# augustgw/early-exit-transformer

Measured on AMD Instinct MI355X. Metric: mel-frames/sec encoder forward (all exits) + summed per-exit CTC loss, d_model=256 12-layer, higher is better.
Workload: dtype fp16x3 (hi/lo-split fp16 MFMA operands, three products per GEMM, fp32 accumulate; v_mfma_f32_16x16x32_f16); 1 GPU; early_conformer ctc 12-layer d_model=256 (6 exits x 2), batch 64/GPU, mel [80 x 1027] -> T'=256, log-normal synthetic mel, random-init weights (BASELINE.json configs[1]); global_batch=64, mel_frames=1027, parallelism=dp1 (utterance-batch shards), precision_mode=f16x3

## Files before the change

early_exit_transformer_amd/csrc/ctc.hip:

```cpp
#include <limits.h>

#include "eec_kernels.h"

namespace eec {

constexpr int kCtcPerLane = 8;
constexpr int kCtcEmpty = -(1 << 20);
constexpr float kCtcTiny = 7.52316385e-37f;
constexpr float kCtcRedo = -1.f;
__host__ __device__ inline int ctc_watch_slack(int Tq) {
  int lg = 0;
  while (((long long)Tq * 2048) >> lg) ++lg;
  return 120 - 26 - lg;
}

#define EEC_DPP_F(old, src, ctrl) \
  __builtin_bit_cast(float, __builtin_amdgcn_update_dpp(__builtin_bit_cast(int, (float)(old)), __builtin_bit_cast(int, (float)(src)), ctrl, 0xf, 0xf, false))
#define EEC_DPP_I(old, src, ctrl) __builtin_amdgcn_update_dpp((int)(old), (int)(src), ctrl, 0xf, 0xf, false)

__device__ __forceinline__ size_t ctc_store_index(int lat, int Tq, int P, int t, int k, int lane) {
  return (((size_t)lat * Tq + t) * (P + 1) + k) * 64 + lane;
}

template <int P, bool STORE>
__global__ __launch_bounds__(64) void ctc_alpha_kernel(const float* __restrict__ logp, const long long* __restrict__ targets,
                                                       const long long* __restrict__ target_len, int B, int Tq, int V,
                                                       int S, int blank, float* __restrict__ nll, float* __restrict__ astore) {
  const int lat = blockIdx.x, b = lat % B, lane = threadIdx.x;
  const float* lp = logp + (size_t)lat * Tq * V;
  const long long len_raw = target_len[b];
  bool bad = len_raw < 0 || len_raw > (long long)S;
  const int len = bad ? 0 : (int)len_raw;
  const int L = 2 * len + 1;
  int label[P];
  bool skip_ok[P], live[P];
#pragma unroll
  for (int i = 0; i < P; ++i) {
    const int s = lane * P + i;
    label[i] = blank;
    skip_ok[i] = false;
    live[i] = s < L;
    if (s < L && (s & 1)) {
      const int k = s >> 1;
      const long long lab = targets[(size_t)b * S + k];
      if (lab < 0 || lab >= (long long)V) bad = true;
      label[i] = (lab < 0 || lab >= (long long)V) ? blank : (int)lab;
      skip_ok[i] = k > 0 && lab != targets[(size_t)b * S + k - 1];
    }
  }
  bad = __any((int)bad) != 0;
  float livef[P];
#pragma unroll
  for (int i = 0; i < P; ++i) {
    livef[i] = live[i] ? 1.f : 0.f;
    asm volatile("" : "+v"(label[i]));
  }
  float alpha[P], lim[P];
  int ex = kCtcEmpty;
  static_assert(P % 2 == 0, "a lane's first state must be a blank");
  int eloss = kCtcEmpty;
#pragma unroll
  for (int i = 0; i < P; ++i) {
    const int s = lane * P + i;
    const float l0 = lp[label[i]];
    alpha[i] = (s < 2 && s < L) ? __expf(l0) : 0.f;
    eloss = ((s < 2 && s < L) & (l0 > -INFINITY) & (alpha[i] < kCtcTiny)) ? 0 : eloss;
    lim[i] = live[i] ? -INFINITY : INFINITY;
  }
  if (lane == 0) ex = 0;
  auto store = [&](int t) {
    if constexpr (STORE) {
#pragma unroll
      for (int i = 0; i < P; ++i) astore[ctc_store_index(lat, Tq, P, t, i, lane)] = alpha[i];
      astore[ctc_store_index(lat, Tq, P, t, P, lane)] = __builtin_bit_cast(float, ex);
    }
  };
  store(0);
  constexpr int kCtcAhead = P <= 4 ? 16 : 8;
  float emit[kCtcAhead][P];
#pragma unroll
  for (int d = 0; d < kCtcAhead; ++d)
#pragma unroll
    for (int i = 0; i < P; ++i) emit[d][i] = lp[(size_t)min(1 + d, Tq - 1) * V + label[i]];
  auto step = [&](const float (&em)[P], bool renorm) {
    float up1 = EEC_DPP_F(0.f, alpha[P - 1], 0x138);
    float up2 = EEC_DPP_F(0.f, alpha[P - 2], 0x138);
    const int ex_up = EEC_DPP_I(ex, ex, 0x138);
    const int ec = max(ex, ex_up);
    const int d_own = max(ex - ec, -200), d_up = max(ex_up - ec, -200);
    const float up1s = ldexpf(up1, d_up), up2s = ldexpf(up2, d_up);
    bool lost = (up1 > 0.f) & (up1s < kCtcTiny);
    up1 = up1s;
    up2 = up2s;
    float cur[P];
#pragma unroll
    for (int i = 0; i < P; ++i) {
      cur[i] = ldexpf(alpha[i], d_own);
      lost |= (alpha[i] > 0.f) & (cur[i] < kCtcTiny);
    }
    ex = ec;
#pragma unroll
    for (int i = 0; i < P; ++i) {
      const float p1 = i >= 1 ? cur[i - 1] : up1;
      const float p2 = i >= 2 ? cur[i - 2] : (i == 1 ? up1 : up2);
      const float sum = cur[i] + p1 + (skip_ok[i] ? p2 : 0.f);
      alpha[i] = sum * (__expf(em[i]) * livef[i]);
      lost |= (sum > 0.f) & (alpha[i] < kCtcTiny) & (em[i] > lim[i]);
    }
    eloss = lost ? max(eloss, ec) : eloss;
    if (renorm) {
      float m = alpha[0];
#pragma unroll
      for (int i = 1; i < P; ++i) m = fmaxf(m, alpha[i]);
      const bool any = m > 0.f;
      const int e = any ? (int)((__builtin_bit_cast(unsigned, m) >> 23) & 0xffu) - 127 : 0;
#pragma unroll
      for (int i = 0; i < P; ++i) alpha[i] = ldexpf(alpha[i], -e);
      ex = any ? ex + e : kCtcEmpty;
    }
  };
  int t0 = 1;
  for (; t0 + kCtcAhead <= Tq; t0 += kCtcAhead) {
#pragma unroll
    for (int d = 0; d < kCtcAhead; ++d) {
      step(emit[d], (d & 1) != 0);
      store(t0 + d);
      const int tn = min(t0 + d + kCtcAhead, Tq - 1);
#pragma unroll
      for (int i = 0; i < P; ++i) emit[d][i] = lp[(size_t)tn * V + label[i]];
    }
  }
#pragma unroll
  for (int d = 0; d < kCtcAhead; ++d)
    if (t0 + d < Tq) {
      step(emit[d], (d & 1) != 0);
      store(t0 + d);
    }
  float tail = 0.f;
#pragma unroll
  for (int i = 0; i < P; ++i) {
    const int s = lane * P + i;
    if (s == L - 1 || s == L - 2) tail += alpha[i];
  }
  bad = bad || __any((int)(tail != tail)) != 0;
  const int e_lane = tail > 0.f ? ex : kCtcEmpty;
  const int e_max = (int)wave_max((float)e_lane);
  const float total = wave_sum(tail > 0.f ? ldexpf(tail, max(e_lane - e_max, -200)) : 0.f);
  const int e_tot = total > 0.f ? e_max + (int)((__builtin_bit_cast(unsigned, total) >> 23) & 0xffu) - 127 : 2 * kCtcEmpty;
  const bool redo = __any((int)(eloss > kCtcEmpty && eloss > e_tot + ctc_watch_slack(Tq))) != 0;
  if (lane == 0)
    nll[lat] = (bad || total != total) ? __builtin_nanf("")
               : redo                  ? -INFINITY
               : (total > 0.f)         ? -(logf(total) + (float)e_max * 0.6931471805599453f)
                                       : INFINITY;
  if constexpr (STORE) {
    if (lane == 0) {
      float* pinfo = astore + ctc_store_index(gridDim.x, Tq, P, 0, 0, 0) + 2 * (size_t)lat;
      pinfo[0] = (bad || total != total) ? __builtin_nanf("") : redo ? kCtcRedo : total;
      pinfo[1] = __builtin_bit_cast(float, e_max);
    }
  }
}

template <int P>
__global__ __launch_bounds__(64) void ctc_beta_kernel(const float* __restrict__ logp, const long long* __restrict__ targets,
                                                      const long long* __restrict__ target_len, int B, int Tq, int V,
                                                      int S, int blank, const float* __restrict__ nll, float* __restrict__ astore) {
  const int lat = blockIdx.x, b = lat % B, lane = threadIdx.x;
  const float* lp = logp + (size_t)lat * Tq * V;
  float* pinfo = astore + ctc_store_index(gridDim.x, Tq, P, 0, 0, 0) + 2 * (size_t)lat;
  if (pinfo[0] < 0.f) return;
  const long long len_raw = target_len[b];
  const int len = (len_raw < 0 || len_raw > (long long)S) ? 0 : (int)len_raw;
  const int L = 2 * len + 1;
  int label[P];
  bool skip_ok[P];
  float livef[P], lim[P];
  bool redo = false;
#pragma unroll
  for (int i = 0; i < P; ++i) {
    const int s = lane * P + i;
    label[i] = blank;
    skip_ok[i] = false;
    livef[i] = s < L ? 1.f : 0.f;
    lim[i] = s < L ? -INFINITY : INFINITY;
    if (s < L && (s & 1)) {
      const int k = s >> 1;
      const long long lab = targets[(size_t)b * S + k];
      label[i] = (lab < 0 || lab >= (long long)V) ? blank : (int)lab;
      skip_ok[i] = k > 0 && lab != targets[(size_t)b * S + k - 1];
    }
    asm volatile("" : "+v"(label[i]));
  }
  bool skip_dn[P];
  {
    const int n0 = EEC_DPP_I(0, (int)skip_ok[0], 0x130), n1 = EEC_DPP_I(0, (int)skip_ok[1], 0x130);
#pragma unroll
    for (int i = 0; i < P; ++i) skip_dn[i] = i + 2 < P ? skip_ok[i + 2] : ((i + 2 - P == 0 ? n0 : n1) != 0);
  }
  const float ptot = pinfo[0];
  const bool usable = ptot > 0.f && ptot < INFINITY;
  const int ishift = usable ? -__builtin_bit_cast(int, pinfo[1]) : 0;
  const float fscale = usable ? 1.0f / ptot : 0.f;
  const int e_ptot = (int)((__builtin_bit_cast(unsigned, ptot) >> 23) & 0xffu) - 127;
  const int e_harm = usable ? -ishift + e_ptot + ctc_watch_slack(Tq) : INT_MAX;
  const int sh_harm = 120 - 26 - 2 + e_ptot;
  float beta[P];
  int eb = kCtcEmpty;
  bool any0 = false;
#pragma unroll
  for (int i = 0; i < P; ++i) {
    const int s = lane * P + i;
    beta[i] = (s < L && (s == L - 1 || s == L - 2)) ? 1.f : 0.f;
    any0 = any0 || beta[i] != 0.f;
  }
  if (any0) eb = 0;
  constexpr int kAhead = P <= 4 ? 8 : 4;
  float emit[kAhead][P], al[kAhead][P + 1];
  auto fetch = [&](int slot, int t) {
    const int tc = max(t, 0);
#pragma unroll
    for (int i = 0; i < P; ++i) emit[slot][i] = lp[(size_t)tc * V + label[i]];
#pragma unroll
    for (int k = 0; k <= P; ++k) al[slot][k] = astore[ctc_store_index(lat, Tq, P, tc, k, lane)];
  };
#pragma unroll
  for (int d = 0; d < kAhead; ++d) fetch(d, Tq - 1 - d);
  auto step = [&](int slot, int t, bool renorm) {
    const int ea = __builtin_bit_cast(int, al[slot][P]);
    const int sh = max(min(ea + eb + ishift, 126), -300);
#pragma unroll
    for (int i = 0; i < P; ++i) {
      const float ab = al[slot][i] * beta[i];
      redo |= (al[slot][i] > 0.f) & (beta[i] > 0.f) & (ab < kCtcTiny) & (sh > sh_harm);
      astore[ctc_store_index(lat, Tq, P, t, i, lane)] = ldexpf(ab * fscale, sh) * livef[i];
    }
    float bw[P];
    bool lost = false;
#pragma unroll
    for (int i = 0; i < P; ++i) {
      bw[i] = beta[i] * (__expf(emit[slot][i]) * livef[i]);
      lost |= (beta[i] > 0.f) & (bw[i] < kCtcTiny) & (emit[slot][i] > lim[i]);
    }
    float dn1 = EEC_DPP_F(0.f, bw[0], 0x130);
    float dn2 = EEC_DPP_F(0.f, bw[1], 0x130);
    const int eb_dn = EEC_DPP_I(kCtcEmpty, eb, 0x130);
    const int ec = max(eb, eb_dn);
    const int d_own = max(eb - ec, -200), d_dn = max(eb_dn - ec, -200);
    const float dn1s = ldexpf(dn1, d_dn), dn2s = ldexpf(dn2, d_dn);
    lost |= ((dn1 > 0.f) & (dn1s < kCtcTiny)) | ((dn2 > 0.f) & (dn2s < kCtcTiny));
    dn1 = dn1s;
    dn2 = dn2s;
#pragma unroll
    for (int i = 0; i < P; ++i) {
      const float sh_own = ldexpf(bw[i], d_own);
      lost |= (bw[i] > 0.f) & (sh_own < kCtcTiny);
      bw[i] = sh_own;
    }
    eb = ec;
    redo |= lost & (ec > e_harm);
#pragma unroll
    for (int i = 0; i < P; ++i) {
      const float n1 = i + 1 < P ? bw[i + 1 < P ? i + 1 : 0] : dn1;
      const float n2 = i + 2 < P ? bw[i + 2 < P ? i + 2 : 0] : (i + 2 - P == 0 ? dn1 : dn2);
      beta[i] = bw[i] + n1 + (skip_dn[i] ? n2 : 0.f);
    }
    if (renorm) {
      float m = beta[0];
#pragma unroll
      for (int i = 1; i < P; ++i) m = fmaxf(m, beta[i]);
      const bool any = m > 0.f;
      const int e = any ? (int)((__builtin_bit_cast(unsigned, m) >> 23) & 0xffu) - 127 : 0;
#pragma unroll
      for (int i = 0; i < P; ++i) beta[i] = ldexpf(beta[i], -e);
      eb = any ? eb + e : kCtcEmpty;
    }
  };
  int t = Tq - 1;
  for (; t - kAhead + 1 >= 0; t -= kAhead) {
#pragma unroll
    for (int d = 0; d < kAhead; ++d) {
      step(d, t - d, (d & 1) != 0);
      fetch(d, t - d - kAhead);
    }
  }
#pragma unroll
  for (int d = 0; d < kAhead; ++d)
    if (t - d >= 0) step(d, t - d, (d & 1) != 0);
  if (usable && __any((int)redo) != 0 && lane == 0) pinfo[0] = kCtcRedo;
}

template <int P>
__global__ __launch_bounds__(256) void ctc_grad_kernel(const float* __restrict__ logp, const long long* __restrict__ targets,
                                                       const long long* __restrict__ target_len, int B, int Tq, int V, int S,
                                                       int blank, const float* __restrict__ nll, const float* __restrict__ astore,
                                                       const float* __restrict__ grad_loss, int n_rows, float* __restrict__ dlogp) {
  __shared__ float bins_all[4][256];
  const int lane = threadIdx.x & 63, w = threadIdx.x >> 6;
  const int row = blockIdx.x * 4 + w;
  float* bins = bins_all[w];
  const bool row_ok = row < n_rows;
  const int lat = row_ok ? row / Tq : 0, t = row_ok ? row - lat * Tq : 0, b = lat % B, e = lat / B;
  *(float4*)(bins + lane * 4) = make_float4(0.f, 0.f, 0.f, 0.f);
  __syncthreads();
  const long long len_raw = target_len[b];
  const int len = (len_raw < 0 || len_raw > (long long)S) ? 0 : (int)len_raw;
  const int L = 2 * len + 1;
  if (row_ok) {
#pragma unroll
    for (int i = 0; i < P; ++i) {
      const int s = lane * P + i;
      if (s < L) {
        int lab = blank;
        if (s & 1) {
          const long long lr = targets[(size_t)b * S + (s >> 1)];
          lab = (lr < 0 || lr >= (long long)V) ? blank : (int)lr;
        }
        atomicAdd(&bins[lab], astore[ctc_store_index(lat, Tq, P, t, i, lane)]);
      }
    }
  }
  __syncthreads();
  if (!row_ok) return;
  const float nl = nll[lat];
  float gs = grad_loss[e] / ((float)B * (float)(len > 0 ? len : 1));
  if (nl != nl) gs = nl;
  else if (!(nl < INFINITY)) gs = 0.f;
  const int c0 = lane * 4;
  if (c0 < V) {
    const size_t off = ((size_t)lat * Tq + t) * V + c0;
    const float4 l = *(const float4*)(logp + off);
    const float4 g = *(const float4*)(bins + c0);
    float4 o;
    o.x = gs * (__expf(l.x) - g.x), o.y = gs * (__expf(l.y) - g.y), o.z = gs * (__expf(l.z) - g.z), o.w = gs * (__expf(l.w) - g.w);
    if (gs == 0.f) o = make_float4(0.f, 0.f, 0.f, 0.f);
    *(float4*)(dlogp + off) = o;
  }
}

constexpr int kCtcWideEmpty = -(1 << 30);

__device__ __forceinline__ void ctc_wide_exp(float l, float& pm, int& k) {
  const float hi = l * 1.44269502f;
  const float lo = fmaf(l, 1.44269502f, -hi) + l * 1.92596299e-8f;
  const float kf = floorf(hi);
  const bool zero = !(l > -3.0e4f);
  pm = zero ? 0.f : exp2f((hi - kf) + lo);
  k = zero ? 0 : (int)kf;
}
__device__ __forceinline__ void ctc_wide_norm(float v, int base, float& m, int& e) {
  const int ex = (int)((__builtin_bit_cast(unsigned, v) >> 23) & 0xffu) - 127;
  const bool any = v > 0.f;
  m = any ? ldexpf(v, -ex) : 0.f;
  e = any ? base + ex : kCtcWideEmpty;
}
__device__ __forceinline__ float ctc_wide_add3(float m0, int e0, float m1, int e1, float m2, int e2, int& ec) {
  ec = max(e0, max(e1, e2));
  return ldexpf(m0, max(e0 - ec, -64)) + ldexpf(m1, max(e1 - ec, -64)) + ldexpf(m2, max(e2 - ec, -64));
}

template <int P, bool GRAD>
__global__ __launch_bounds__(64) void ctc_wide_kernel(const float* __restrict__ logp, const long long* __restrict__ targets,
                                                      const long long* __restrict__ target_len, int B, int Tq, int V, int S,
                                                      int blank, float* __restrict__ nll, float* __restrict__ astore) {
  const int lat = blockIdx.x, b = lat % B, lane = threadIdx.x;
  if constexpr (GRAD) {
    if (!(astore[ctc_store_index(gridDim.x, Tq, P, 0, 0, 0) + 2 * (size_t)lat] < 0.f)) return;
  } else {
    if (!(nll[lat] == -INFINITY)) return;
  }
  const float* lp = logp + (size_t)lat * Tq * V;
  int* estore = GRAD ? (int*)(astore + ctc_store_index(gridDim.x, Tq, P, 0, 0, 0) + 2 * (size_t)gridDim.x) : nullptr;
  const long long len_raw = target_len[b];
  const int len = (len_raw < 0 || len_raw > (long long)S) ? 0 : (int)len_raw;
  const int L = 2 * len + 1;
  int label[P];
  bool skip_ok[P], live[P];
#pragma unroll
  for (int i = 0; i < P; ++i) {
    const int s = lane * P + i;
    label[i] = blank;
    skip_ok[i] = false;
    live[i] = s < L;
    if (s < L && (s & 1)) {
      const int k = s >> 1;
      const long long lab = targets[(size_t)b * S + k];
      label[i] = (lab < 0 || lab >= (long long)V) ? blank : (int)lab;
      skip_ok[i] = k > 0 && lab != targets[(size_t)b * S + k - 1];
    }
  }
  float am[P];
  int ae[P];
#pragma unroll
  for (int i = 0; i < P; ++i) {
    const int s = lane * P + i;
    float pm;
    int k;
    ctc_wide_exp(lp[label[i]], pm, k);
    ctc_wide_norm((s < 2 && s < L) ? pm : 0.f, k, am[i], ae[i]);
  }
  auto store = [&](int t) {
    if constexpr (GRAD) {
#pragma unroll
      for (int i = 0; i < P; ++i) {
        astore[ctc_store_index(lat, Tq, P, t, i, lane)] = am[i];
        estore[(((size_t)lat * Tq + t) * P + i) * 64 + lane] = ae[i];
      }
    }
  };
  store(0);
  constexpr int kAhead = 4;
  float emit[kAhead][P];
#pragma unroll
  for (int d = 0; d < kAhead; ++d)
#pragma unroll
    for (int i = 0; i < P; ++i) emit[d][i] = lp[(size_t)min(1 + d, Tq - 1) * V + label[i]];
  for (int t0 = 1; t0 < Tq; t0 += kAhead)
#pragma unroll
  for (int d = 0; d < kAhead; ++d) {
    const int t = t0 + d;
    if (t >= Tq) break;
    const float u1m = EEC_DPP_F(0.f, am[P - 1], 0x138), u2m = EEC_DPP_F(0.f, am[P - 2], 0x138);
    const int u1e = EEC_DPP_I(kCtcWideEmpty, ae[P - 1], 0x138), u2e = EEC_DPP_I(kCtcWideEmpty, ae[P - 2], 0x138);
    float nm[P];
    int ne[P];
#pragma unroll
    for (int i = 0; i < P; ++i) {
      const float p1m = i >= 1 ? am[i >= 1 ? i - 1 : 0] : u1m;
      const int p1e = i >= 1 ? ae[i >= 1 ? i - 1 : 0] : u1e;
      float p2m = i >= 2 ? am[i >= 2 ? i - 2 : 0] : (i == 1 ? u1m : u2m);
      int p2e = i >= 2 ? ae[i >= 2 ? i - 2 : 0] : (i == 1 ? u1e : u2e);
      if (!skip_ok[i]) p2m = 0.f, p2e = kCtcWideEmpty;
      float pm;
      int k, ec;
      ctc_wide_exp(emit[d][i], pm, k);
      const float sum = ctc_wide_add3(am[i], ae[i], p1m, p1e, p2m, p2e, ec);
      ctc_wide_norm(live[i] ? sum * pm : 0.f, ec + k, nm[i], ne[i]);
    }
#pragma unroll
    for (int i = 0; i < P; ++i) {
      am[i] = nm[i], ae[i] = ne[i];
      emit[d][i] = lp[(size_t)min(t + kAhead, Tq - 1) * V + label[i]];
    }
    store(t);
  }
  float tm = 0.f;
  int te = kCtcWideEmpty;
#pragma unroll
  for (int i = 0; i < P; ++i) {
    const int s = lane * P + i;
    if (s == L - 1 || s == L - 2) {
      int ec;
      tm = ctc_wide_add3(tm, te, am[i], ae[i], 0.f, kCtcWideEmpty, ec);
      te = tm > 0.f ? ec : kCtcWideEmpty;
    }
  }
  int e_max = te;
#pragma unroll
  for (int off = 32; off >= 1; off >>= 1) e_max = max(e_max, __shfl_xor(e_max, off, 64));
  float total = ldexpf(tm, max(te - e_max, -64));
#pragma unroll
  for (int off = 32; off >= 1; off >>= 1) total += __shfl_xor(total, off, 64);
  float mt;
  int et;
  ctc_wide_norm(total, e_max, mt, et);
  if constexpr (!GRAD) {
    if (lane == 0) nll[lat] = total > 0.f ? -(logf(mt) + (float)et * 0.6931471805599453f) : INFINITY;
    return;
  } else {
    if (!(total > 0.f)) return;
    bool skip_dn[P];
    {
      int n0 = __shfl_down((int)skip_ok[0], 1, 64), n1 = __shfl_down((int)skip_ok[1], 1, 64);
      if (lane == 63) n0 = n1 = 0;
#pragma unroll
      for (int i = 0; i < P; ++i) skip_dn[i] = i + 2 < P ? skip_ok[i + 2 < P ? i + 2 : 0] : ((i + 2 - P == 0 ? n0 : n1) != 0);
    }
    const float inv = 1.0f / mt;
    float bm[P];
    int be[P];
#pragma unroll
    for (int i = 0; i < P; ++i) {
      const int s = lane * P + i;
      const bool last = s < L && (s == L - 1 || s == L - 2);
      bm[i] = last ? 1.f : 0.f;
      be[i] = last ? 0 : kCtcWideEmpty;
    }
    for (int t = Tq - 1; t >= 0; --t) {
      float wm[P];
      int we[P];
#pragma unroll
      for (int i = 0; i < P; ++i) {
        const size_t ia = ctc_store_index(lat, Tq, P, t, i, lane);
        const float a_m = astore[ia];
        const int a_e = estore[(((size_t)lat * Tq + t) * P + i) * 64 + lane];
        const bool nz = a_m > 0.f && bm[i] > 0.f;
        const int sh = nz ? min(max(a_e + be[i] - et, -200), 126) : 0;
        astore[ia] = nz ? ldexpf(a_m * bm[i] * inv, sh) : 0.f;
        float pm;
        int k;
        ctc_wide_exp(lp[(size_t)t * V + label[i]], pm, k);
        ctc_wide_norm(live[i] ? bm[i] * pm : 0.f, be[i] + k, wm[i], we[i]);
      }
      float d1m = __shfl_down(wm[0], 1, 64), d2m = __shfl_down(wm[1], 1, 64);
      int d1e = __shfl_down(we[0], 1, 64), d2e = __shfl_down(we[1], 1, 64);
      if (lane == 63) d1m = d2m = 0.f, d1e = d2e = kCtcWideEmpty;
#pragma unroll
      for (int i = 0; i < P; ++i) {
        const float n1m = i + 1 < P ? wm[i + 1 < P ? i + 1 : 0] : d1m;
        const int n1e = i + 1 < P ? we[i + 1 < P ? i + 1 : 0] : d1e;
        float n2m = i + 2 < P ? wm[i + 2 < P ? i + 2 : 0] : (i + 2 - P == 0 ? d1m : d2m);
        int n2e = i + 2 < P ? we[i + 2 < P ? i + 2 : 0] : (i + 2 - P == 0 ? d1e : d2e);
        if (!skip_dn[i]) n2m = 0.f, n2e = kCtcWideEmpty;
        int ec;
        const float sum = ctc_wide_add3(wm[i], we[i], n1m, n1e, n2m, n2e, ec);
        ctc_wide_norm(sum, ec, bm[i], be[i]);
      }
    }
  }
}

int ctc_states_per_lane(int S) {
  if (2 * S + 1 <= 64 * 2) return 2;
  if (2 * S + 1 <= 64 * 4) return 4;
  if (2 * S + 1 <= 64 * kCtcPerLane) return kCtcPerLane;
  return 0;
}

size_t ctc_store_floats(int E, int B, int Tq, int S) {
  const int P = ctc_states_per_lane(S);
  return P ? (size_t)E * B * Tq * (P + 1) * 64 + 2 * (size_t)E * B + (size_t)E * B * Tq * P * 64 : 0;
}

hipError_t launch_ctc_backward(const float* logp, const long long* targets, const long long* target_len, int E, int B, int Tq,
                               int V, int S, int blank, const float* nll, float* astore, const float* grad_loss, float* dlogp,
                               hipStream_t st) {
  const int P = ctc_states_per_lane(S), n_rows = E * B * Tq;
  if (!P || V > 256 || V % 4) return hipErrorInvalidValue;
#define EEC_CTC_BWD(P_)                                                                                                      \
  hipLaunchKernelGGL(ctc_beta_kernel<P_>, dim3(E * B), dim3(64), 0, st, logp, targets, target_len, B, Tq, V, S, blank, nll,  \
                     astore);                                                                                               \
  hipLaunchKernelGGL((ctc_wide_kernel<P_, true>), dim3(E * B), dim3(64), 0, st, logp, targets, target_len, B, Tq, V, S,      \
                     blank, (float*)nullptr, astore);                                                                        \
  hipLaunchKernelGGL(ctc_grad_kernel<P_>, dim3((n_rows + 3) / 4), dim3(256), 0, st, logp, targets, target_len, B, Tq, V, S,  \
                     blank, nll, astore, grad_loss, n_rows, dlogp);
  if (P == 2) {
    EEC_CTC_BWD(2)
  } else if (P == 4) {
    EEC_CTC_BWD(4)
  } else {
    EEC_CTC_BWD(kCtcPerLane)
  }
#undef EEC_CTC_BWD
  return hipGetLastError();
}

__global__ void ctc_reduce_kernel(const float* nll, const long long* target_len, int B, float* out) {
  const int e = blockIdx.x, lane = threadIdx.x;
  float s = 0.f;
  for (int b0 = 0; b0 < B; b0 += 64) {
    const int b = b0 + lane;
    float term = 0.f;
    if (b < B) {
      float v = nll[e * B + b];
      if (isinf(v)) v = 0.f;
      const long long l = target_len[b] > 0 ? target_len[b] : 1;
      term = v / (float)l;
    }
    const int n = min(64, B - b0);
    for (int i = 0; i < n; ++i) s += __shfl(term, i, 64);
  }
  if (lane == 0) out[e] = s / (float)B;
}

hipError_t launch_ctc_loss(const float* logp, const long long* targets, const long long* target_len, int E, int B, int Tq,
                           int V, int S, int blank, float* nll, float* out, float* astore, hipStream_t st) {
  const int P = ctc_states_per_lane(S);
  if (!P) return hipErrorInvalidValue;
#define EEC_CTC_FWD(P_)                                                                                                        \
  if (astore)                                                                                                                  \
    hipLaunchKernelGGL((ctc_alpha_kernel<P_, true>), dim3(E * B), dim3(64), 0, st, logp, targets, target_len, B, Tq, V, S,     \
                       blank, nll, astore);                                                                                    \
  else                                                                                                                         \
    hipLaunchKernelGGL((ctc_alpha_kernel<P_, false>), dim3(E * B), dim3(64), 0, st, logp, targets, target_len, B, Tq, V, S,    \
                       blank, nll, astore);                                                                                    \
  hipLaunchKernelGGL((ctc_wide_kernel<P_, false>), dim3(E * B), dim3(64), 0, st, logp, targets, target_len, B, Tq, V, S,       \
                     blank, nll, astore);
  if (P == 2) {
    EEC_CTC_FWD(2)
  } else if (P == 4) {
    EEC_CTC_FWD(4)
  } else {
    EEC_CTC_FWD(kCtcPerLane)
  }
#undef EEC_CTC_FWD
  hipError_t e = hipGetLastError();
  if (e != hipSuccess) return e;
  hipLaunchKernelGGL(ctc_reduce_kernel, dim3(E), dim3(64), 0, st, nll, target_len, B, out);
  return hipGetLastError();
}

__global__ __launch_bounds__(256) void logsoftmax_bwd_kernel(const float* __restrict__ logp, const float* __restrict__ g, int M, int V,
                                                             float* __restrict__ dlogits) {
  const int lane = threadIdx.x & 63, row = blockIdx.x * 4 + (threadIdx.x >> 6);
  if (row >= M) return;
  const int c0 = lane * 4;
  float4 gv = make_float4(0.f, 0.f, 0.f, 0.f), lv = gv;
  if (c0 < V) {
    gv = *(const float4*)(g + (size_t)row * V + c0);
    lv = *(const float4*)(logp + (size_t)row * V + c0);
  }
  const float sum = wave_sum(gv.x + gv.y + gv.z + gv.w);
  if (c0 < V)
    *(float4*)(dlogits + (size_t)row * V + c0) = make_float4(gv.x - __expf(lv.x) * sum, gv.y - __expf(lv.y) * sum,
                                                             gv.z - __expf(lv.z) * sum, gv.w - __expf(lv.w) * sum);
}

hipError_t launch_logsoftmax_backward(const float* logp, const float* g, int M, int V, float* dlogits, hipStream_t st) {
  if (V > 256 || V % 4) return hipErrorInvalidValue;
  hipLaunchKernelGGL(logsoftmax_bwd_kernel, dim3((M + 3) / 4), dim3(256), 0, st, logp, g, M, V, dlogits);
  return hipGetLastError();
}

}
```

Measured before the change: 19.54 million mel-frames/s.

## Add bidirectional alpha/beta CTC kernel for loss-only forward path

When no alpha store is needed, the forward CTC loss now launches a single 128-thread kernel. One wavefront runs the alpha recursion up to the midpoint while the other runs the beta recursion down from the end, and the two halves are joined through shared memory. This roughly halves the serial time-step chain per utterance and drops the second wide-kernel launch, at the cost of twice the threads per block and a different NaN/invalid handling path. The step logic is also refactored into shared helpers, the beta step now uses DPP instead of shuffles, and a raw exp2 builtin replaces exp2f.

```diff
diff --git a/early_exit_transformer_amd/csrc/ctc.hip b/early_exit_transformer_amd/csrc/ctc.hip
--- a/early_exit_transformer_amd/csrc/ctc.hip
+++ b/early_exit_transformer_amd/csrc/ctc.hip
@@ -339,13 +339,14 @@
 }
 
 constexpr int kCtcWideEmpty = -(1 << 30);
+constexpr int kCtcWideAhead = 4;
 
 __device__ __forceinline__ void ctc_wide_exp(float l, float& pm, int& k) {
   const float hi = l * 1.44269502f;
   const float lo = fmaf(l, 1.44269502f, -hi) + l * 1.92596299e-8f;
   const float kf = floorf(hi);
-  const bool zero = !(l > -3.0e4f);
-  pm = zero ? 0.f : exp2f((hi - kf) + lo);
+  const bool zero = l <= -3.0e4f;
+  pm = zero ? 0.f : __builtin_amdgcn_exp2f((hi - kf) + lo);
   k = zero ? 0 : (int)kf;
 }
 __device__ __forceinline__ void ctc_wide_norm(float v, int base, float& m, int& e) {
@@ -358,6 +359,133 @@
   ec = max(e0, max(e1, e2));
   return ldexpf(m0, max(e0 - ec, -64)) + ldexpf(m1, max(e1 - ec, -64)) + ldexpf(m2, max(e2 - ec, -64));
 }
+
+template <int P>
+__device__ __forceinline__ bool ctc_wide_labels(const long long* __restrict__ targets, const long long* __restrict__ target_len, int b,
+                                                int V, int S, int blank, int lane, int (&label)[P], bool (&skip_ok)[P],
+                                                bool (&live)[P], int& L) {
+  const long long len_raw = target_len[b];
+  bool bad = len_raw < 0 || len_raw > (long long)S;
+  const int len = bad ? 0 : (int)len_raw;
+  L = 2 * len + 1;
+#pragma unroll
+  for (int i = 0; i < P; ++i) {
+    const int s = lane * P + i;
+    label[i] = blank;
+    skip_ok[i] = false;
+    live[i] = s < L;
+    if (s < L && (s & 1)) {
+      const int k = s >> 1;
+      const long long lab = targets[(size_t)b * S + k];
+      bad = bad || lab < 0 || lab >= (long long)V;
+      label[i] = (lab < 0 || lab >= (long long)V) ? blank : (int)lab;
+      skip_ok[i] = k > 0 && lab != targets[(size_t)b * S + k - 1];
+    }
+    asm volatile("" : "+v"(label[i]));
+  }
+  return bad;
+}
+
+template <int P>
+__device__ __forceinline__ void ctc_wide_skip_dn(const bool (&skip_ok)[P], int lane, bool (&skip_dn)[P]) {
+  int n0 = __shfl_down((int)skip_ok[0], 1, 64), n1 = __shfl_down((int)skip_ok[1], 1, 64);
+  if (lane == 63) n0 = n1 = 0;
+#pragma unroll
+  for (int i = 0; i < P; ++i) skip_dn[i] = i + 2 < P ? skip_ok[i + 2 < P ? i + 2 : 0] : ((i + 2 - P == 0 ? n0 : n1) != 0);
+}
+
+template <int P>
+__device__ __forceinline__ void ctc_wide_alpha0(const float* __restrict__ lp, const int (&label)[P], int L, int lane, float (&am)[P],
+                                                int (&ae)[P], bool& nan) {
+#pragma unroll
+  for (int i = 0; i < P; ++i) {
+    const int s = lane * P + i;
+    const float l0 = lp[label[i]];
+    float pm;
+    int k;
+    ctc_wide_exp(l0, pm, k);
+    ctc_wide_norm((s < 2 && s < L) ? pm : 0.f, k, am[i], ae[i]);
+    nan |= s < L && l0 != l0;
+  }
+}
+template <int P>
+__device__ __forceinline__ void ctc_wide_beta_last(int L, int lane, float (&bm)[P], int (&be)[P]) {
+#pragma unroll
+  for (int i = 0; i < P; ++i) {
+    const int s = lane * P + i;
+    const bool last = s < L && (s == L - 1 || s == L - 2);
+    bm[i] = last ? 1.f : 0.f;
+    be[i] = last ? 0 : kCtcWideEmpty;
+  }
+}
+
+template <int P>
+__device__ __forceinline__ void ctc_wide_alpha_step(float (&am)[P], int (&ae)[P], const float (&em)[P], const bool (&skip_ok)[P],
+                                                    const bool (&live)[P], bool& nan) {
+  const float u1m = EEC_DPP_F(0.f, am[P - 1], 0x138), u2m = EEC_DPP_F(0.f, am[P - 2], 0x138);
+  const int u1e = EEC_DPP_I(kCtcWideEmpty, ae[P - 1], 0x138), u2e = EEC_DPP_I(kCtcWideEmpty, ae[P - 2], 0x138);
+  float nm[P];
+  int ne[P];
+#pragma unroll
+  for (int i = 0; i < P; ++i) {
+    const float p1m = i >= 1 ? am[i >= 1 ? i - 1 : 0] : u1m;
+    const int p1e = i >= 1 ? ae[i >= 1 ? i - 1 : 0] : u1e;
+    float p2m = i >= 2 ? am[i >= 2 ? i - 2 : 0] : (i == 1 ? u1m : u2m);
+    int p2e = i >= 2 ? ae[i >= 2 ? i - 2 : 0] : (i == 1 ? u1e : u2e);
+    if (!skip_ok[i]) p2m = 0.f, p2e = kCtcWideEmpty;
+    float pm;
+    int k, ec;
+    ctc_wide_exp(em[i], pm, k);
+    const float sum = ctc_wide_add3(am[i], ae[i], p1m, p1e, p2m, p2e, ec);
+    const float v = live[i] ? sum * pm : 0.f;
+    nan |= v != v;
+    ctc_wide_norm(v, ec + k, nm[i], ne[i]);
+  }
+#pragma unroll
+  for (int i = 0; i < P; ++i) am[i] = nm[i], ae[i] = ne[i];
+}
+
+template <int P>
+__device__ __forceinline__ void ctc_wide_beta_step(float (&bm)[P], int (&be)[P], const float (&em)[P], const bool (&skip_dn)[P],
+                                                   bool& nan) {
+  float wm[P];
+  int we[P];
+#pragma unroll
+  for (int i = 0; i < P; ++i) {
+    float pm;
+    int k;
+    ctc_wide_exp(em[i], pm, k);
+    const float v = bm[i] * pm;
+    nan |= v != v;
+    wm[i] = v > 0.f ? v : 0.f;
+    we[i] = v > 0.f ? be[i] + k : kCtcWideEmpty;
+  }
+  const float d1m = EEC_DPP_F(0.f, wm[0], 0x130), d2m = EEC_DPP_F(0.f, wm[1], 0x130);
+  const int d1e = EEC_DPP_I(kCtcWideEmpty, we[0], 0x130), d2e = EEC_DPP_I(kCtcWideEmpty, we[1], 0x130);
+#pragma unroll
+  for (int i = 0; i < P; ++i) {
+    const float n1m = i + 1 < P ? wm[i + 1 < P ? i + 1 : 0] : d1m;
+    const int n1e = i + 1 < P ? we[i + 1 < P ? i + 1 : 0] : d1e;
+    float n2m = i + 2 < P ? wm[i + 2 < P ? i + 2 : 0] : (i + 2 - P == 0 ? d1m : d2m);
+    int n2e = i + 2 < P ? we[i + 2 < P ? i + 2 : 0] : (i + 2 - P == 0 ? d1e : d2e);
+    if (!skip_dn[i]) n2m = 0.f, n2e = kCtcWideEmpty;
+    int ec;
+    const float sum = ctc_wide_add3(wm[i], we[i], n1m, n1e, n2m, n2e, ec);
+    ctc_wide_norm(sum, ec, bm[i], be[i]);
+  }
+}
+
+__device__ __forceinline__ float ctc_wide_total(float tm, int te, float& mt, int& et) {
+  int e_max = te;
+#pragma unroll
+  for (int off = 32; off >= 1; off >>= 1) e_max = max(e_max, __shfl_xor(e_max, off, 64));
+  float total = ldexpf(tm, max(te - e_max, -64));
+#pragma unroll
+  for (int off = 32; off >= 1; off >>= 1) total += __shfl_xor(total, off, 64);
+  ctc_wide_norm(total, e_max, mt, et);
+  return total;
+}
+
 
 template <int P, bool GRAD>
 __global__ __launch_bounds__(64) void ctc_wide_kernel(const float* __restrict__ logp, const long long* __restrict__ targets,
@@ -371,34 +499,12 @@
   }
   const float* lp = logp + (size_t)lat * Tq * V;
   int* estore = GRAD ? (int*)(astore + ctc_store_index(gridDim.x, Tq, P, 0, 0, 0) + 2 * (size_t)gridDim.x) : nullptr;
-  const long long len_raw = target_len[b];
-  const int len = (len_raw < 0 || len_raw > (long long)S) ? 0 : (int)len_raw;
-  const int L = 2 * len + 1;
-  int label[P];
-  bool skip_ok[P], live[P];
-#pragma unroll
-  for (int i = 0; i < P; ++i) {
-    const int s = lane * P + i;
-    label[i] = blank;
-    skip_ok[i] = false;
-    live[i] = s < L;
-    if (s < L && (s & 1)) {
-      const int k = s >> 1;
-      const long long lab = targets[(size_t)b * S + k];
-      label[i] = (lab < 0 || lab >= (long long)V) ? blank : (int)lab;
-      skip_ok[i] = k > 0 && lab != targets[(size_t)b * S + k - 1];
-    }
-  }
+  int label[P], L;
+  bool skip_ok[P], live[P], nan = false;
+  ctc_wide_labels<P>(targets, target_len, b, V, S, blank, lane, label, skip_ok, live, L);
   float am[P];
   int ae[P];
-#pragma unroll
-  for (int i = 0; i < P; ++i) {
-    const int s = lane * P + i;
-    float pm;
-    int k;
-    ctc_wide_exp(lp[label[i]], pm, k);
-    ctc_wide_norm((s < 2 && s < L) ? pm : 0.f, k, am[i], ae[i]);
-  }
+  ctc_wide_alpha0<P>(lp, label, L, lane, am, ae, nan);
   auto store = [&](int t) {
     if constexpr (GRAD) {
 #pragma unroll
@@ -409,39 +515,19 @@
     }
   };
   store(0);
-  constexpr int kAhead = 4;
-  float emit[kAhead][P];
-#pragma unroll
-  for (int d = 0; d < kAhead; ++d)
+  float emit[kCtcWideAhead][P];
+#pragma unroll
+  for (int d = 0; d < kCtcWideAhead; ++d)
 #pragma unroll
     for (int i = 0; i < P; ++i) emit[d][i] = lp[(size_t)min(1 + d, Tq - 1) * V + label[i]];
-  for (int t0 = 1; t0 < Tq; t0 += kAhead)
-#pragma unroll
-  for (int d = 0; d < kAhead; ++d) {
+  for (int t0 = 1; t0 < Tq; t0 += kCtcWideAhead)
+#pragma unroll
+  for (int d = 0; d < kCtcWideAhead; ++d) {
     const int t = t0 + d;
     if (t >= Tq) break;
-    const float u1m = EEC_DPP_F(0.f, am[P - 1], 0x138), u2m = EEC_DPP_F(0.f, am[P - 2], 0x138);
-    const int u1e = EEC_DPP_I(kCtcWideEmpty, ae[P - 1], 0x138), u2e = EEC_DPP_I(kCtcWideEmpty, ae[P - 2], 0x138);
-    float nm[P];
-    int ne[P];
-#pragma unroll
-    for (int i = 0; i < P; ++i) {
-      const float p1m = i >= 1 ? am[i >= 1 ? i - 1 : 0] : u1m;
-      const int p1e = i >= 1 ? ae[i >= 1 ? i - 1 : 0] : u1e;
-      float p2m = i >= 2 ? am[i >= 2 ? i - 2 : 0] : (i == 1 ? u1m : u2m);
-      int p2e = i >= 2 ? ae[i >= 2 ? i - 2 : 0] : (i == 1 ? u1e : u2e);
-      if (!skip_ok[i]) p2m = 0.f, p2e = kCtcWideEmpty;
-      float pm;
-      int k, ec;
-      ctc_wide_exp(emit[d][i], pm, k);
-      const float sum = ctc_wide_add3(am[i], ae[i], p1m, p1e, p2m, p2e, ec);
-      ctc_wide_norm(live[i] ? sum * pm : 0.f, ec + k, nm[i], ne[i]);
-    }
-#pragma unroll
-    for (int i = 0; i < P; ++i) {
-      am[i] = nm[i], ae[i] = ne[i];
-      emit[d][i] = lp[(size_t)min(t + kAhead, Tq - 1) * V + label[i]];
-    }
+    ctc_wide_alpha_step<P>(am, ae, emit[d], skip_ok, live, nan);
+#pragma unroll
+    for (int i = 0; i < P; ++i) emit[d][i] = lp[(size_t)min(t + kCtcWideAhead, Tq - 1) * V + label[i]];
     store(t);
   }
   float tm = 0.f;
@@ -455,40 +541,22 @@
       te = tm > 0.f ? ec : kCtcWideEmpty;
     }
   }
-  int e_max = te;
-#pragma unroll
-  for (int off = 32; off >= 1; off >>= 1) e_max = max(e_max, __shfl_xor(e_max, off, 64));
-  float total = ldexpf(tm, max(te - e_max, -64));
-#pragma unroll
-  for (int off = 32; off >= 1; off >>= 1) total += __shfl_xor(total, off, 64);
   float mt;
   int et;
-  ctc_wide_norm(total, e_max, mt, et);
+  const float total = ctc_wide_total(tm, te, mt, et);
   if constexpr (!GRAD) {
     if (lane == 0) nll[lat] = total > 0.f ? -(logf(mt) + (float)et * 0.6931471805599453f) : INFINITY;
     return;
   } else {
     if (!(total > 0.f)) return;
     bool skip_dn[P];
-    {
-      int n0 = __shfl_down((int)skip_ok[0], 1, 64), n1 = __shfl_down((int)skip_ok[1], 1, 64);
-      if (lane == 63) n0 = n1 = 0;
-#pragma unroll
-      for (int i = 0; i < P; ++i) skip_dn[i] = i + 2 < P ? skip_ok[i + 2 < P ? i + 2 : 0] : ((i + 2 - P == 0 ? n0 : n1) != 0);
-    }
+    ctc_wide_skip_dn<P>(skip_ok, lane, skip_dn);
     const float inv = 1.0f / mt;
     float bm[P];
     int be[P];
-#pragma unroll
-    for (int i = 0; i < P; ++i) {
-      const int s = lane * P + i;
-      const bool last = s < L && (s == L - 1 || s == L - 2);
-      bm[i] = last ? 1.f : 0.f;
-      be[i] = last ? 0 : kCtcWideEmpty;
-    }
+    ctc_wide_beta_last<P>(L, lane, bm, be);
     for (int t = Tq - 1; t >= 0; --t) {
-      float wm[P];
-      int we[P];
+      float em[P];
 #pragma unroll
       for (int i = 0; i < P; ++i) {
         const size_t ia = ctc_store_index(lat, Tq, P, t, i, lane);
@@ -497,27 +565,96 @@
         const bool nz = a_m > 0.f && bm[i] > 0.f;
         const int sh = nz ? min(max(a_e + be[i] - et, -200), 126) : 0;
         astore[ia] = nz ? ldexpf(a_m * bm[i] * inv, sh) : 0.f;
-        float pm;
-        int k;
-        ctc_wide_exp(lp[(size_t)t * V + label[i]], pm, k);
-        ctc_wide_norm(live[i] ? bm[i] * pm : 0.f, be[i] + k, wm[i], we[i]);
+        em[i] = lp[(size_t)t * V + label[i]];
       }
-      float d1m = __shfl_down(wm[0], 1, 64), d2m = __shfl_down(wm[1], 1, 64);
-      int d1e = __shfl_down(we[0], 1, 64), d2e = __shfl_down(we[1], 1, 64);
-      if (lane == 63) d1m = d2m = 0.f, d1e = d2e = kCtcWideEmpty;
-#pragma unroll
-      for (int i = 0; i < P; ++i) {
-        const float n1m = i + 1 < P ? wm[i + 1 < P ? i + 1 : 0] : d1m;
-        const int n1e = i + 1 < P ? we[i + 1 < P ? i + 1 : 0] : d1e;
-        float n2m = i + 2 < P ? wm[i + 2 < P ? i + 2 : 0] : (i + 2 - P == 0 ? d1m : d2m);
-        int n2e = i + 2 < P ? we[i + 2 < P ? i + 2 : 0] : (i + 2 - P == 0 ? d1e : d2e);
-        if (!skip_dn[i]) n2m = 0.f, n2e = kCtcWideEmpty;
-        int ec;
-        const float sum = ctc_wide_add3(wm[i], we[i], n1m, n1e, n2m, n2e, ec);
-        ctc_wide_norm(sum, ec, bm[i], be[i]);
+      ctc_wide_beta_step<P>(bm, be, em, skip_dn, nan);
+    }
+  }
+}
+
+template <int P>
+__global__ __launch_bounds__(128) void ctc_bidir_kernel(const float* __restrict__ logp, const long long* __restrict__ targets,
+                                                        const long long* __restrict__ target_len, int B, int Tq, int V, int S,
+                                                        int blank, float* __restrict__ nll) {
+  __shared__ float join_m[P][64];
+  __shared__ int join_e[P][64];
+  __shared__ int join_nan;
+  const int lat = blockIdx.x, b = lat % B, lane = threadIdx.x & 63;
+  const bool down = __builtin_amdgcn_readfirstlane((int)threadIdx.x >> 6) != 0;
+  const float* lp = logp + (size_t)lat * Tq * V;
+  int label[P], L;
+  bool skip_ok[P], live[P], nan = false;
+  const bool bad = ctc_wide_labels<P>(targets, target_len, b, V, S, blank, lane, label, skip_ok, live, L);
+  const int mid = (Tq - 1) / 2;
+  constexpr int kAhead = P <= 4 ? 8 : 4;
+  float xm[P], emit[kAhead][P];
+  int xe[P];
+  if (!down) {
+    ctc_wide_alpha0<P>(lp, label, L, lane, xm, xe, nan);
+#pragma unroll
+    for (int d = 0; d < kAhead; ++d)
+#pragma unroll
+      for (int i = 0; i < P; ++i) emit[d][i] = lp[(size_t)min(1 + d, Tq - 1) * V + label[i]];
+    int t0 = 1;
+    for (; t0 + kAhead - 1 <= mid; t0 += kAhead) {
+#pragma unroll
+      for (int d = 0; d < kAhead; ++d) {
+#pragma unroll
+        for (int i = 0; i < P; ++i) asm volatile("" : "+v"(emit[d][i]) : "v"(xm[0]));
+        ctc_wide_alpha_step<P>(xm, xe, emit[d], skip_ok, live, nan);
+        const int tn = min(t0 + d + kAhead, Tq - 1);
+#pragma unroll
+        for (int i = 0; i < P; ++i) emit[d][i] = lp[(size_t)tn * V + label[i]];
       }
     }
-  }
+#pragma unroll
+    for (int d = 0; d < kAhead; ++d)
+      if (t0 + d <= mid) ctc_wide_alpha_step<P>(xm, xe, emit[d], skip_ok, live, nan);
+  } else {
+    bool skip_dn[P];
+    ctc_wide_skip_dn<P>(skip_ok, lane, skip_dn);
+    ctc_wide_beta_last<P>(L, lane, xm, xe);
+#pragma unroll
+    for (int d = 0; d < kAhead; ++d)
+#pragma unroll
+      for (int i = 0; i < P; ++i) emit[d][i] = lp[(size_t)max(Tq - 1 - d, 0) * V + label[i]];
+    int t0 = Tq - 1;
+    for (; t0 - kAhead + 1 > mid; t0 -= kAhead) {
+#pragma unroll
+      for (int d = 0; d < kAhead; ++d) {
+        ctc_wide_beta_step<P>(xm, xe, emit[d], skip_dn, nan);
+        const int tn = max(t0 - d - kAhead, 0);
+#pragma unroll
+        for (int i = 0; i < P; ++i) emit[d][i] = lp[(size_t)tn * V + label[i]];
+      }
+    }
+#pragma unroll
+    for (int d = 0; d < kAhead; ++d)
+      if (t0 - d > mid) ctc_wide_beta_step<P>(xm, xe, emit[d], skip_dn, nan);
+#pragma unroll
+    for (int i = 0; i < P; ++i) join_m[i][lane] = xm[i], join_e[i][lane] = xe[i];
+    const bool any_nan = __any((int)nan) != 0;
+    if (lane == 0) join_nan = (int)any_nan;
+  }
+  __syncthreads();
+  if (down) return;
+  float tm = 0.f;
+  int te = kCtcWideEmpty;
+#pragma unroll
+  for (int i = 0; i < P; ++i) {
+    float pm;
+    int pe, ec;
+    ctc_wide_norm(xm[i] * join_m[i][lane], 0, pm, pe);
+    pe = pm > 0.f ? pe + xe[i] + join_e[i][lane] : kCtcWideEmpty;
+    tm = ctc_wide_add3(tm, te, pm, pe, 0.f, kCtcWideEmpty, ec);
+    te = tm > 0.f ? ec : kCtcWideEmpty;
+  }
+  float mt;
+  int et;
+  const float total = ctc_wide_total(tm, te, mt, et);
+  const bool invalid = join_nan != 0 || __any((int)(bad || nan)) != 0;
+  if (lane == 0)
+    nll[lat] = invalid ? __builtin_nanf("") : total > 0.f ? -(logf(mt) + (float)et * 0.6931471805599453f) : INFINITY;
 }
 
 int ctc_states_per_lane(int S) {
@@ -578,14 +715,15 @@
   const int P = ctc_states_per_lane(S);
   if (!P) return hipErrorInvalidValue;
 #define EEC_CTC_FWD(P_)                                                                                                        \
-  if (astore)                                                                                                                  \
+  if (astore) {                                                                                                                \
     hipLaunchKernelGGL((ctc_alpha_kernel<P_, true>), dim3(E * B), dim3(64), 0, st, logp, targets, target_len, B, Tq, V, S,     \
                        blank, nll, astore);                                                                                    \
-  else                                                                                                                         \
-    hipLaunchKernelGGL((ctc_alpha_kernel<P_, false>), dim3(E * B), dim3(64), 0, st, logp, targets, target_len, B, Tq, V, S,    \
+    hipLaunchKernelGGL((ctc_wide_kernel<P_, false>), dim3(E * B), dim3(64), 0, st, logp, targets, target_len, B, Tq, V, S,     \
                        blank, nll, astore);                                                                                    \
-  hipLaunchKernelGGL((ctc_wide_kernel<P_, false>), dim3(E * B), dim3(64), 0, st, logp, targets, target_len, B, Tq, V, S,       \
-                     blank, nll, astore);
+  } else {                                                                                                                     \
+    hipLaunchKernelGGL(ctc_bidir_kernel<P_>, dim3(E * B), dim3(128), 0, st, logp, targets, target_len, B, Tq, V, S, blank,     \
+                       nll);                                                                                                   \
+  }
   if (P == 2) {
     EEC_CTC_FWD(2)
   } else if (P == 4) {
```

Result: faster. 19.92 million mel-frames/s, median of 6 (+1.9%).
